# strongbeamsprout/gloria-nlp-project

Hardware: AMD Instinct MI355X
Metric: image-text pairs/sec (whole node), imagenome_pretrain bs=256 (higher is better)
Workload: dtype bf16

## Files before the change

gloria-nlp-project_amd/csrc/glr_attn.hip:

```cpp
#include "glr_attn_common.h"

namespace {

__global__ void __launch_bounds__(AT_NT) k_attn_fwd(AttnParams p) {
  extern __shared__ __attribute__((aligned(16))) unsigned char smem[];
  const int tid = threadIdx.x, lane = tid & 63, wave = tid >> 6, l31 = lane & 31, h = lane >> 5;
  const int bh = blockIdx.x, b = bh / p.nh, hd = bh % p.nh;
  const int L = p.L, tp = p.tp, lk = (L + 15) & ~15, kt = lk >> 4, nkb = (L + 31) >> 5;
  unsigned char* Qs = smem;
  unsigned char* Ks = Qs + 128 * AT_RP;
  unsigned char* Vt = Ks + 128 * AT_RP;
  unsigned char* Ps = smem;
  float* kb = reinterpret_cast<float*>(Vt + 64 * tp);
  const size_t base = (size_t)b * L * p.ld + (size_t)hd * 64;
  {
    uint4 rq[4], rk[4], rv[4];
    tile_load(p.q + base, p.ld, L, rq, tid);
    tile_load(p.k + base, p.ld, L, rk, tid);
    tile_load(p.v + base, p.ld, L, rv, tid);
    tile_store_rows(rq, Qs, tid);
    tile_store_rows(rk, Ks, tid);
    tile_store_transposed(rv, lk, Vt, tp, tid);
  }
  if (tid < 128) kb[tid] = (tid < L && (p.key_mask == nullptr || p.key_mask[(size_t)b * L + tid] != 0)) ? 0.f : -INFINITY;
  __syncthreads();
  const int row0 = 32 * wave;
  f32x16 acc[4];
#pragma unroll
  for (int j = 0; j < 4; ++j) zero16(acc[j]);
  if (row0 < L) gemm_rows64(acc, Qs, row0, Ks, nkb, l31, h);
  __syncthreads();
  if (row0 >= L) return;
  float kbv[4];
#pragma unroll
  for (int j = 0; j < 4; ++j) kbv[j] = kb[32 * j + l31];
  const bool drop = p.p_drop > 0.f;
  const unsigned thr16 = drop ? (unsigned)(p.p_drop * 65536.f + 0.5f) : 0u;
  const float inv_keep = drop ? 1.f / (1.f - p.p_drop) : 1.f;
  const float sl = p.scale * AT_LOG2E;
  unsigned char* slab = Ps + wave * 32 * AT_SP;
  unsigned mw0 = 0u, mw1 = 0u;
  unsigned hk0, hk1;
  hash_key(p, hk0, hk1);
#pragma unroll
  for (int q = 0; q < 16; ++q) {
    const int r = acc_row(q, h);
    float v[4], m = -INFINITY;
#pragma unroll
    for (int j = 0; j < 4; ++j) { v[j] = __builtin_fmaf(acc[j][q], sl, kbv[j]); m = fmaxf(m, v[j]); }
    m = half_max(m);
    const float ms = m == -INFINITY ? 0.f : m;
    float e[4], s = 0.f;
#pragma unroll
    for (int j = 0; j < 4; ++j) { e[j] = __builtin_amdgcn_exp2f(v[j] - ms); s += e[j]; }
    s = half_sum(s);
    const float inv = s > 0.f ? 1.f / s : 0.f;
    if (l31 == 0) p.lse[(size_t)bh * 128 + row0 + r] = (ms + __builtin_amdgcn_logf(fmaxf(s, 1e-37f))) * (1.f / AT_LOG2E);
    unsigned r01 = 0u, r23 = 0u;
    if (drop) {
      const unsigned ctr = (((unsigned)bh * 128u + (unsigned)(row0 + r)) * 32u + (unsigned)l31) * 2u;
      r01 = hash32(ctr, hk0, hk1);
      r23 = hash32(ctr + 1u, hk0, hk1);
    }
    const unsigned r16[4] = {r01 & 0xffffu, r01 >> 16, r23 & 0xffffu, r23 >> 16};
#pragma unroll
    for (int j = 0; j < 4; ++j) {
      const bool keepb = !drop || r16[j] >= thr16;
      if (drop) {
        const unsigned long long word = __ballot(keepb);
        if (lane == q * 4 + j) { mw0 = (unsigned)word; mw1 = (unsigned)(word >> 32); }
      }
      const float pd = keepb ? e[j] * inv * inv_keep : 0.f;
      *reinterpret_cast<unsigned short*>(slab + r * AT_SP + (32 * j + l31) * 2) = f2bf(pd);
    }
  }
  if (drop) {
    const int q = lane >> 2, j = lane & 3;
    const int r0 = row0 + acc_row(q, 0);
    p.keep[((size_t)bh * 128 + r0) * 4 + j] = mw0;
    p.keep[((size_t)bh * 128 + r0 + 4) * 4 + j] = mw1;
  }
  f32x16 out[2];
  zero16(out[0]); zero16(out[1]);
  gemm_tokens(out, slab, Vt, tp, kt, l31, h);
  store_rows(out, slab, tp, p.o + (size_t)b * L * p.ld_o + (size_t)hd * 64, p.ld_o, row0, L, lane, l31, h);
}

__global__ void __launch_bounds__(AT_NT, 2) k_attn_bwd_q(AttnParams p) {
  extern __shared__ __attribute__((aligned(16))) unsigned char smem[];
  const int tid = threadIdx.x, lane = tid & 63, wave = tid >> 6, l31 = lane & 31, h = lane >> 5;
  const int bh = blockIdx.x, b = bh / p.nh, hd = bh % p.nh;
  const int L = p.L, tp = p.tp, lk = (L + 15) & ~15, kt = lk >> 4, nkb = (L + 31) >> 5;
  unsigned char* Ks = smem;
  unsigned char* Vs = Ks + 128 * AT_RP;
  unsigned char* Kt = Vs + 128 * AT_RP;
  unsigned char* Ps = smem;
  float* kb = reinterpret_cast<float*>(Kt + 64 * tp);
  float* lse = kb + 128;
  float* delta = lse + 128;
  unsigned* keep = reinterpret_cast<unsigned*>(delta + 128);
  const size_t base = (size_t)b * L * p.ld + (size_t)hd * 64, base_o = (size_t)b * L * p.ld_o + (size_t)hd * 64;
  const bool drop = p.p_drop > 0.f;
  const int row0 = 32 * wave;
  const bool active = row0 < L;
  bf16x8 fq[4], fg[4];
  {
    uint4 rk[4], rv[4];
    bf16x8 fo[4];
    tile_load(p.k + base, p.ld, L, rk, tid);
    tile_load(p.v + base, p.ld, L, rv, tid);
    frag_rows_load(p.q + base, p.ld, row0 + l31, L, h, fq);
    frag_rows_load(p.d_o + base_o, p.ld_o, row0 + l31, L, h, fg);
    frag_rows_load(p.o + base_o, p.ld_o, row0 + l31, L, h, fo);
    if (tid < 128) {
      kb[tid] = (tid < L && (p.key_mask == nullptr || p.key_mask[(size_t)b * L + tid] != 0)) ? 0.f : -INFINITY;
      lse[tid] = tid < L ? p.lse[(size_t)bh * 128 + tid] * AT_LOG2E : 0.f;
    }
    for (int i = tid; i < 512; i += AT_NT) keep[i] = (drop && (i >> 2) < L) ? p.keep[(size_t)bh * 512 + i] : 0xffffffffu;
    tile_store_rows(rk, Ks, tid);
    tile_store_rows(rv, Vs, tid);
    tile_store_transposed(rk, lk, Kt, tp, tid);
    float d = 0.f;
#pragma unroll
    for (int ks = 0; ks < 4; ++ks) d += dot8(__builtin_bit_cast(uint4, fg[ks]), __builtin_bit_cast(uint4, fo[ks]));
    d += __shfl_xor(d, 32, 64);
    if (h == 0) delta[row0 + l31] = d;
  }
  __syncthreads();
  f32x16 acc[4], acc2[4], out[2];
#pragma unroll
  for (int j = 0; j < 4; ++j) { zero16(acc[j]); zero16(acc2[j]); }
  if (active) {
    gemm_frag64(acc, fq, Ks, nkb, l31, h);
    gemm_frag64(acc2, fg, Vs, nkb, l31, h);
  }
  __syncthreads();
  if (!active) return;
  const float inv_keep = drop ? 1.f / (1.f - p.p_drop) : 1.f;
  const float sl = p.scale * AT_LOG2E;
  unsigned char* slab = Ps + wave * 32 * AT_SP;
  {
    float kbv[4];
#pragma unroll
    for (int j = 0; j < 4; ++j) kbv[j] = kb[32 * j + l31];
#pragma unroll
    for (int q = 0; q < 16; ++q) {
      const int r = acc_row(q, h);
      const float lr = lse[row0 + r], dl = delta[row0 + r];
      const uint4 kw = *reinterpret_cast<const uint4*>(keep + (row0 + r) * 4);
      const unsigned kwj[4] = {kw.x, kw.y, kw.z, kw.w};
#pragma unroll
      for (int j = 0; j < 4; ++j) {
        const float pr = __builtin_amdgcn_exp2f(__builtin_fmaf(acc[j][q], sl, kbv[j]) - lr);
        const float dp = ((kwj[j] >> l31) & 1u) ? acc2[j][q] * inv_keep : 0.f;
        *reinterpret_cast<unsigned short*>(slab + r * AT_SP + (32 * j + l31) * 2) = f2bf(pr * (dp - dl) * p.scale);
      }
    }
  }
  zero16(out[0]); zero16(out[1]);
  gemm_tokens(out, slab, Kt, tp, kt, l31, h);
  store_rows(out, slab, tp, p.dq + base, p.ld, row0, L, lane, l31, h);
}

__global__ void __launch_bounds__(AT_NT, 2) k_attn_bwd_kv(AttnParams p) {
  extern __shared__ __attribute__((aligned(16))) unsigned char smem[];
  const int tid = threadIdx.x, lane = tid & 63, wave = tid >> 6, l31 = lane & 31, h = lane >> 5;
  const int bh = blockIdx.x, b = bh / p.nh, hd = bh % p.nh;
  const int L = p.L, tp = p.tp, lk = (L + 15) & ~15, kt = lk >> 4, nkb = (L + 31) >> 5;
  unsigned char* Qs = smem;
  unsigned char* Gs = Qs + 128 * AT_RP;
  unsigned char* Qt = Gs + 128 * AT_RP;
  unsigned char* Gt = Qt + 64 * tp;
  unsigned char* Ps = smem;
  float* kb = reinterpret_cast<float*>(Gt + 64 * tp);
  float* lse = kb + 128;
  float* delta = lse + 128;
  unsigned* keep = reinterpret_cast<unsigned*>(delta + 256);
  const size_t base = (size_t)b * L * p.ld + (size_t)hd * 64, base_o = (size_t)b * L * p.ld_o + (size_t)hd * 64;
  const bool drop = p.p_drop > 0.f;
  const int row0 = 32 * wave;
  const bool active = row0 < L;
  bf16x8 fk[4], fv[4];
  {
    uint4 rq[4], rg[4], ro[4];
    tile_load(p.q + base, p.ld, L, rq, tid);
    tile_load(p.d_o + base_o, p.ld_o, L, rg, tid);
    tile_load(p.o + base_o, p.ld_o, L, ro, tid);
    frag_rows_load(p.k + base, p.ld, row0 + l31, L, h, fk);
    frag_rows_load(p.v + base, p.ld, row0 + l31, L, h, fv);
    if (tid < 128) {
      kb[tid] = (tid < L && (p.key_mask == nullptr || p.key_mask[(size_t)b * L + tid] != 0)) ? 0.f : -INFINITY;
      lse[tid] = tid < L ? p.lse[(size_t)bh * 128 + tid] * AT_LOG2E : 0.f;
    }
    for (int i = tid; i < 512; i += AT_NT) keep[i] = (drop && (i >> 2) < L) ? p.keep[(size_t)bh * 512 + i] : 0xffffffffu;
    tile_store_rows(rq, Qs, tid);
    tile_store_rows(rg, Gs, tid);
    tile_store_transposed(rq, lk, Qt, tp, tid);
    tile_store_transposed(rg, lk, Gt, tp, tid);
    delta[tid] = (dot8(rg[0], ro[0]) + dot8(rg[1], ro[1])) + (dot8(rg[2], ro[2]) + dot8(rg[3], ro[3]));
  }
  __syncthreads();
  f32x16 acc[4], acc2[4], out[2];
#pragma unroll
  for (int j = 0; j < 4; ++j) { zero16(acc[j]); zero16(acc2[j]); }
  float lq[4], dq_[4], kbk16[16];
  unsigned kwq[4];
  if (active) {
    gemm_frag64(acc, fk, Qs, nkb, l31, h);
    gemm_frag64(acc2, fv, Gs, nkb, l31, h);
  }
#pragma unroll
  for (int j = 0; j < 4; ++j) {
    lq[j] = lse[32 * j + l31];
    dq_[j] = delta[32 * j + l31] + delta[128 + 32 * j + l31];
    kwq[j] = keep[(32 * j + l31) * 4 + wave];
  }
#pragma unroll
  for (int q = 0; q < 16; ++q) kbk16[q] = kb[row0 + acc_row(q, h)];
  __syncthreads();
  if (!active) return;
  const float inv_keep = drop ? 1.f / (1.f - p.p_drop) : 1.f;
  const float sl = p.scale * AT_LOG2E;
  unsigned char* slab = Ps + wave * 32 * AT_SP;
#pragma unroll
  for (int q = 0; q < 16; ++q) {
    const int r = acc_row(q, h);
#pragma unroll
    for (int j = 0; j < 4; ++j) {
      const float pr = __builtin_amdgcn_exp2f(__builtin_fmaf(acc[j][q], sl, kbk16[q]) - lq[j]);
      const bool keepb = (kwq[j] >> r) & 1u;
      *reinterpret_cast<unsigned short*>(slab + r * AT_SP + (32 * j + l31) * 2) = f2bf(keepb ? pr * inv_keep : 0.f);
      const float dp = keepb ? acc2[j][q] * inv_keep : 0.f;
      acc2[j][q] = pr * (dp - dq_[j]) * p.scale;
    }
  }
  zero16(out[0]); zero16(out[1]);
  gemm_tokens(out, slab, Gt, tp, kt, l31, h);
  {
    f32x16 dvv[2] = {out[0], out[1]};
#pragma unroll
    for (int q = 0; q < 16; ++q) {
      const int r = acc_row(q, h);
#pragma unroll
      for (int j = 0; j < 4; ++j) *reinterpret_cast<unsigned short*>(slab + r * AT_SP + (32 * j + l31) * 2) = f2bf(acc2[j][q]);
    }
    zero16(out[0]); zero16(out[1]);
    gemm_tokens(out, slab, Qt, tp, kt, l31, h);
    store_rows(out, slab, tp, p.dk + base, p.ld, row0, L, lane, l31, h);
    store_rows(dvv, slab, tp, p.dv + base, p.ld, row0, L, lane, l31, h);
  }
}

size_t attn_lds_fwd(int L) { return (size_t)2 * 128 * AT_RP + (size_t)64 * attn_tp(L) + 512; }
size_t attn_lds_bwd_q(int L) { return (size_t)2 * 128 * AT_RP + (size_t)64 * attn_tp(L) + 3 * 512 + 2048; }
size_t attn_lds_bwd_kv(int L) { return (size_t)2 * 128 * AT_RP + (size_t)2 * 64 * attn_tp(L) + 4 * 512 + 2048; }
size_t attn_lds_bwd(int L) { return attn_lds_bwd_kv(L) > attn_lds_bwd_q(L) ? attn_lds_bwd_kv(L) : attn_lds_bwd_q(L); }

}

extern "C" int glr_attn_max_tokens(int backward) {
  for (int L = 128; L > 0; L -= 16)
    if ((backward ? attn_lds_bwd(L) : attn_lds_fwd(L)) <= 160 * 1024) return L;
  return 0;
}

extern "C" int glr_attn_fwd(const void* q, const void* k, const void* v, const uint8_t* key_mask, int B, int n_heads, int L, int ld,
                            int ld_o, float scale, float p_drop, unsigned long long seed, unsigned long long offset,
                            const unsigned long long* rng_cell, void* o, float* lse, uint32_t* keep, void* stream) {
  AttnParams p;
  const int rc = attn_fill(p, q, k, v, key_mask, B, n_heads, L, ld, ld_o, scale, p_drop, seed, offset, 128);
  if (rc != GLR_OK) return rc;
  if (!o || !lse || (p_drop > 0.f && !keep) || L > glr_attn_max_tokens(0)) return GLR_EINVAL;
  p.o = (unsigned short*)o; p.lse = lse; p.keep = keep; p.rng = rng_cell;
  const int lds = (int)attn_lds_fwd(L);
  static GlrLdsAttr lds_fwd;
  if (glr_ensure_lds(lds_fwd, (const void*)k_attn_fwd, lds) != GLR_OK) return GLR_ELAUNCH;
  hipLaunchKernelGGL(k_attn_fwd, dim3(B * n_heads), dim3(AT_NT), lds, (hipStream_t)stream, p);
  GLR_CHECK_LAUNCH();
  return GLR_OK;
}

extern "C" int glr_attn_bwd(const void* q, const void* k, const void* v, const void* o, const void* d_o, const uint8_t* key_mask,
                            const float* lse, const uint32_t* keep, int B, int n_heads, int L, int ld, int ld_o, float scale, float p_drop,
                            void* dq, void* dk, void* dv, void* stream) {
  AttnParams p;
  const int rc = attn_fill(p, q, k, v, key_mask, B, n_heads, L, ld, ld_o, scale, p_drop, 0, 0, 128);
  if (rc != GLR_OK) return rc;
  if (!o || !d_o || !lse || !dq || !dk || !dv || (p_drop > 0.f && !keep) || L > glr_attn_max_tokens(1)) return GLR_EINVAL;
  p.o = (unsigned short*)const_cast<void*>(o); p.d_o = (const unsigned short*)d_o; p.lse = const_cast<float*>(lse);
  p.keep = const_cast<unsigned*>(keep); p.dq = (unsigned short*)dq; p.dk = (unsigned short*)dk; p.dv = (unsigned short*)dv;
  const int lds_q = (int)attn_lds_bwd_q(L), lds_kv = (int)attn_lds_bwd_kv(L);
  static GlrLdsAttr lds_bq, lds_bkv;
  if (glr_ensure_lds(lds_bq, (const void*)k_attn_bwd_q, lds_q) != GLR_OK) return GLR_ELAUNCH;
  if (glr_ensure_lds(lds_bkv, (const void*)k_attn_bwd_kv, lds_kv) != GLR_OK) return GLR_ELAUNCH;
  hipLaunchKernelGGL(k_attn_bwd_q, dim3(B * n_heads), dim3(AT_NT), lds_q, (hipStream_t)stream, p);
  GLR_CHECK_LAUNCH();
  hipLaunchKernelGGL(k_attn_bwd_kv, dim3(B * n_heads), dim3(AT_NT), lds_kv, (hipStream_t)stream, p);
  GLR_CHECK_LAUNCH();
  return GLR_OK;
}
```

gloria-nlp-project_amd/csrc/glr_attn_common.h:

```cpp
#pragma once
#include "glr_common.h"

namespace {

constexpr int AT_NT = 256;
constexpr int AT_RP = 144;
constexpr int AT_SP = 272;
constexpr float AT_LOG2E = 1.4426950408889634f;

struct AttnParams {
  const unsigned short* q; const unsigned short* k; const unsigned short* v;
  const unsigned char* key_mask;
  int B, nh, L, ld, ld_o;
  float scale, p_drop;
  unsigned seed_lo, seed_hi, off_lo, off_hi;
  const unsigned long long* rng;
  unsigned short* o;
  float* lse;
  unsigned* keep;
  const unsigned short* d_o;
  unsigned short* dq; unsigned short* dk; unsigned short* dv;
  int tp;
};

__device__ __forceinline__ unsigned mix32(unsigned x) {
  x ^= x >> 16; x *= 0x7feb352du; x ^= x >> 15; x *= 0x846ca68bu; x ^= x >> 16;
  return x;
}
__device__ __forceinline__ unsigned hash32(unsigned ctr, unsigned k0, unsigned k1) { return mix32(mix32(ctr ^ k0) + k1); }

template <int CTRL>
__device__ __forceinline__ float dpp(float v) {
  return __builtin_bit_cast(float, __builtin_amdgcn_update_dpp(0, __builtin_bit_cast(int, v), CTRL, 0xf, 0xf, true));
}
__device__ __forceinline__ float half_max(float v) {
  v = fmaxf(v, dpp<0xB1>(v));
  v = fmaxf(v, dpp<0x4E>(v));
  v = fmaxf(v, dpp<0x141>(v));
  v = fmaxf(v, dpp<0x140>(v));
  return fmaxf(v, __shfl_xor(v, 16, 64));
}
__device__ __forceinline__ float half_sum(float v) {
  v += dpp<0xB1>(v);
  v += dpp<0x4E>(v);
  v += dpp<0x141>(v);
  v += dpp<0x140>(v);
  return v + __shfl_xor(v, 16, 64);
}

__device__ __forceinline__ bf16x8 ldf(const unsigned char* p) { return __builtin_bit_cast(bf16x8, *reinterpret_cast<const uint4*>(p)); }
__device__ __forceinline__ void mma(const bf16x8& a, const bf16x8& b, f32x16& c) { c = __builtin_amdgcn_mfma_f32_32x32x16_bf16(a, b, c, 0, 0, 0); }
__device__ __forceinline__ void zero16(f32x16& a) {
#pragma unroll
  for (int q = 0; q < 16; ++q) a[q] = 0.f;
}
__device__ __forceinline__ int acc_row(int q, int h) { return (q & 3) + 8 * (q >> 2) + 4 * h; }

__device__ __forceinline__ void tile_load(const unsigned short* g, int ld, int L, uint4 (&r)[4], int tid) {
#pragma unroll
  for (int t = 0; t < 4; ++t) {
    const int i = tid + AT_NT * t, row = i & 127, pc = i >> 7;
    r[t] = make_uint4(0u, 0u, 0u, 0u);
    if (row < L) r[t] = *reinterpret_cast<const uint4*>(g + (size_t)row * ld + pc * 8);
  }
}
__device__ __forceinline__ void tile_store_rows(const uint4 (&r)[4], unsigned char* dst, int tid) {
#pragma unroll
  for (int t = 0; t < 4; ++t) {
    const int i = tid + AT_NT * t, row = i & 127, pc = i >> 7;
    *reinterpret_cast<uint4*>(dst + row * AT_RP + pc * 16) = r[t];
  }
}
__device__ __forceinline__ void tile_store_transposed(const uint4 (&r)[4], int lk, unsigned char* dst, int tp, int tid) {
#pragma unroll
  for (int t = 0; t < 4; ++t) {
    const int i = tid + AT_NT * t, row = i & 127, pc = i >> 7;
    if (row < lk) {
      const unsigned w[4] = {r[t].x, r[t].y, r[t].z, r[t].w};
#pragma unroll
      for (int e = 0; e < 4; ++e) {
        *reinterpret_cast<unsigned short*>(dst + (pc * 8 + 2 * e) * tp + row * 2) = (unsigned short)(w[e] & 0xffffu);
        *reinterpret_cast<unsigned short*>(dst + (pc * 8 + 2 * e + 1) * tp + row * 2) = (unsigned short)(w[e] >> 16);
      }
    }
  }
}
__device__ __forceinline__ float dot8(const uint4 a, const uint4 c) {
  const unsigned aw[4] = {a.x, a.y, a.z, a.w}, cw[4] = {c.x, c.y, c.z, c.w};
  float d = 0.f;
#pragma unroll
  for (int e = 0; e < 4; ++e) {
    d = __builtin_fmaf(__uint_as_float(aw[e] << 16), __uint_as_float(cw[e] << 16), d);
    d = __builtin_fmaf(__uint_as_float(aw[e] & 0xffff0000u), __uint_as_float(cw[e] & 0xffff0000u), d);
  }
  return d;
}
__device__ __forceinline__ void gemm_rows64(f32x16 (&acc)[4], const unsigned char* A, int arow0, const unsigned char* Bm, int nblk,
                                            int l31, int h) {
#pragma unroll
  for (int ks = 0; ks < 4; ++ks) {
    const bf16x8 fa = ldf(A + (arow0 + l31) * AT_RP + ks * 32 + h * 16);
#pragma unroll
    for (int j = 0; j < 4; ++j)
      if (j < nblk) mma(fa, ldf(Bm + (32 * j + l31) * AT_RP + ks * 32 + h * 16), acc[j]);
  }
}
__device__ __forceinline__ void gemm_tokens(f32x16 (&out)[2], const unsigned char* slab, const unsigned char* Bt, int tp, int kt,
                                            int l31, int h) {
  for (int ks = 0; ks < kt; ++ks) {
    const bf16x8 fa = ldf(slab + l31 * AT_SP + ks * 32 + h * 16);
#pragma unroll
    for (int c = 0; c < 2; ++c) mma(fa, ldf(Bt + (32 * c + l31) * tp + ks * 32 + h * 16), out[c]);
  }
}
__device__ __forceinline__ void store_rows(const f32x16 (&out)[2], unsigned char* slab, int tp, unsigned short* g, int ld, int row0, int L,
                                           int lane, int l31, int h) {
#pragma unroll
  for (int c = 0; c < 2; ++c)
#pragma unroll
    for (int q = 0; q < 16; ++q)
      *reinterpret_cast<unsigned short*>(slab + acc_row(q, h) * AT_SP + (32 * c + l31) * 2) = f2bf(out[c][q]);
#pragma unroll
  for (int t = 0; t < 4; ++t) {
    const int i = lane + 64 * t, row = i >> 3, pc = i & 7;
    if (row0 + row < L)
      *reinterpret_cast<uint4*>(g + (size_t)(row0 + row) * ld + pc * 8) = *reinterpret_cast<const uint4*>(slab + row * AT_SP + pc * 16);
  }
}

__device__ __forceinline__ void frag_rows_load(const unsigned short* g, int ld, int row, int L, int h, bf16x8 (&f)[4]) {
#pragma unroll
  for (int ks = 0; ks < 4; ++ks) {
    uint4 v = make_uint4(0u, 0u, 0u, 0u);
    if (row < L) v = *reinterpret_cast<const uint4*>(g + (size_t)row * ld + ks * 16 + h * 8);
    f[ks] = __builtin_bit_cast(bf16x8, v);
  }
}
__device__ __forceinline__ void gemm_frag64(f32x16 (&acc)[4], const bf16x8 (&fa)[4], const unsigned char* Bm, int nblk, int l31, int h) {
#pragma unroll
  for (int ks = 0; ks < 4; ++ks)
#pragma unroll
    for (int j = 0; j < 4; ++j)
      if (j < nblk) mma(fa[ks], ldf(Bm + (32 * j + l31) * AT_RP + ks * 32 + h * 16), acc[j]);
}

__device__ __forceinline__ void hash_key(const AttnParams& p, unsigned& hk0, unsigned& hk1) {
  unsigned sd_lo = p.seed_lo, sd_hi = p.seed_hi, of_lo = p.off_lo, of_hi = p.off_hi;
  if (p.rng != nullptr) {
    const unsigned long long s = p.rng[0], o = p.rng[1] + (((unsigned long long)p.off_hi << 32) | p.off_lo);
    sd_lo = (unsigned)s; sd_hi = (unsigned)(s >> 32); of_lo = (unsigned)o; of_hi = (unsigned)(o >> 32);
  }
  hk0 = sd_lo ^ (of_lo * 0x9E3779B9u); hk1 = sd_hi ^ (of_hi * 0x85EBCA6Bu) ^ 0xC2B2AE35u;
}

inline int attn_tp(int L) { return 2 * ((L + 15) & ~15) + 16; }

inline int attn_fill(AttnParams& p, const void* q, const void* k, const void* v, const unsigned char* key_mask, int B, int nh, int L, int ld,
                     int ld_o, float scale, float p_drop, unsigned long long seed, unsigned long long offset, int max_L) {
  if (!q || !k || !v || B <= 0 || nh <= 0 || L <= 0 || L > max_L || ld < nh * 64 || ld % 8 != 0 || ld_o < nh * 64 || ld_o % 8 != 0)
    return GLR_EINVAL;
  if (p_drop < 0.f || p_drop >= 1.f) return GLR_EINVAL;
  p.q = (const unsigned short*)q; p.k = (const unsigned short*)k; p.v = (const unsigned short*)v; p.key_mask = key_mask;
  p.B = B; p.nh = nh; p.L = L; p.ld = ld; p.ld_o = ld_o; p.scale = scale; p.p_drop = p_drop;
  p.seed_lo = (unsigned)seed; p.seed_hi = (unsigned)(seed >> 32); p.off_lo = (unsigned)offset; p.off_hi = (unsigned)(offset >> 32);
  p.rng = nullptr;
  p.o = nullptr; p.lse = nullptr; p.keep = nullptr; p.d_o = nullptr; p.dq = p.dk = p.dv = nullptr;
  p.tp = attn_tp(L < 128 ? L : 128);
  return GLR_OK;
}

}
```

gloria-nlp-project_amd/csrc/glr_attn_long.hip:

```cpp
#include "glr_attn_common.h"

namespace {

constexpr int AL_MAX = 512;
constexpr int AL_TP = 272;

__device__ __forceinline__ float key_bias(const AttnParams& p, int b, int key) {
  return (key < p.L && (p.key_mask == nullptr || p.key_mask[(size_t)b * p.L + key] != 0)) ? 0.f : -INFINITY;
}
__device__ __forceinline__ void key_bias_fill(const AttnParams& p, int b, int Lp, float* kb, int* last64, int tid) {
  for (int i0 = 0; i0 < Lp; i0 += AT_NT) {
    const int i = i0 + tid;
    const float v = i < Lp ? key_bias(p, b, i) : -INFINITY;
    const unsigned long long live = __ballot(v == 0.f);
    if (i < Lp) {
      kb[i] = v;
      if ((tid & 63) == 0) last64[i >> 6] = live ? 63 - __builtin_clzll(live) : -1;
    }
  }
}
__device__ __forceinline__ int live_subblocks(const int* last64, int c) {
  const int lo = last64[2 * c], hi = last64[2 * c + 1];
  return hi >= 0 ? (64 + hi) / 32 + 1 : lo >= 0 ? lo / 32 + 1 : 0;
}
__device__ __forceinline__ void uniform_branch() { asm volatile(""); }

__device__ __forceinline__ void keep_load(const AttnParams& p, int bh, int Lp, int qb, int kc, unsigned (&w)[2], int tid) {
#pragma unroll
  for (int t = 0; t < 2; ++t) {
    const int i = tid + AT_NT * t, row = qb * 128 + (i >> 2);
    w[t] = (p.p_drop > 0.f && row < p.L) ? p.keep[((size_t)bh * Lp + row) * (Lp >> 5) + kc * 4 + (i & 3)] : 0xffffffffu;
  }
}

__global__ void __launch_bounds__(AT_NT, 2) k_attn_long_fwd(AttnParams p) {
  extern __shared__ __attribute__((aligned(16))) unsigned char smem[];
  const int tid = threadIdx.x, lane = tid & 63, wave = tid >> 6, l31 = lane & 31, h = lane >> 5;
  const int L = p.L, Lp = (L + 127) & ~127, nb = Lp >> 7;
  const int bh = blockIdx.x / nb, qb = blockIdx.x % nb, b = bh / p.nh, hd = bh % p.nh;
  unsigned char* Ks = smem;
  unsigned char* Vt = Ks + 128 * AT_RP;
  unsigned char* Ps = Vt + 64 * AL_TP;
  float* kb = reinterpret_cast<float*>(Ps + 128 * AT_SP);
  int* last64 = reinterpret_cast<int*>(kb + AL_MAX);
  const size_t base = (size_t)b * L * p.ld + (size_t)hd * 64;
  const int row0 = qb * 128 + 32 * wave;
  const bool active = row0 < L;
  bf16x8 fq[4];
  frag_rows_load(p.q + base, p.ld, row0 + l31, L, h, fq);
  key_bias_fill(p, b, Lp, kb, last64, tid);
  __syncthreads();
  const float sl = p.scale * AT_LOG2E;
  float m[16], s[16];
#pragma unroll
  for (int q = 0; q < 16; ++q) { m[q] = -INFINITY; s[q] = 0.f; }
  for (int c = 0; c < nb; ++c) {
    const int ne = live_subblocks(last64, c);
    if (ne == 0) continue;
    uint4 rk[4];
    tile_load(p.k + base + (size_t)c * 128 * p.ld, p.ld, min(L - c * 128, 32 * ne), rk, tid);
    __syncthreads();
    tile_store_rows(rk, Ks, tid);
    __syncthreads();
    if (active) {
      f32x16 acc[4];
#pragma unroll
      for (int j = 0; j < 4; ++j) zero16(acc[j]);
      gemm_frag64(acc, fq, Ks, ne, l31, h);
      float kbv[4];
#pragma unroll
      for (int j = 0; j < 4; ++j) kbv[j] = kb[c * 128 + 32 * j + l31];
#pragma unroll
      for (int q = 0; q < 16; ++q) {
        float v[4], mb = -INFINITY;
#pragma unroll
        for (int j = 0; j < 4; ++j)
          if (j < ne) { uniform_branch(); v[j] = __builtin_fmaf(acc[j][q], sl, kbv[j]); mb = fmaxf(mb, v[j]); }
        const float mn = fmaxf(m[q], half_max(mb));
        const float ms = mn == -INFINITY ? 0.f : mn;
        float e = 0.f;
#pragma unroll
        for (int j = 0; j < 4; ++j)
          if (j < ne) { uniform_branch(); e += __builtin_amdgcn_exp2f(v[j] - ms); }
        s[q] = __builtin_fmaf(s[q], __builtin_amdgcn_exp2f(m[q] - ms), half_sum(e));
        m[q] = mn;
      }
    }
  }
  const bool drop = p.p_drop > 0.f;
  const unsigned thr16 = drop ? (unsigned)(p.p_drop * 65536.f + 0.5f) : 0u;
  const float inv_keep = drop ? 1.f / (1.f - p.p_drop) : 1.f;
  if (active) {
#pragma unroll
    for (int q = 0; q < 16; ++q) {
      const float ms = m[q] == -INFINITY ? 0.f : m[q];
      if (l31 == 0)
        p.lse[(size_t)bh * Lp + row0 + acc_row(q, h)] = (ms + __builtin_amdgcn_logf(fmaxf(s[q], 1e-37f))) * (1.f / AT_LOG2E);
      m[q] = ms;
      s[q] = s[q] > 0.f ? 1.f / s[q] : 0.f;
    }
  }
  unsigned hk0, hk1;
  hash_key(p, hk0, hk1);
  unsigned char* slab = Ps + wave * 32 * AT_SP;
  f32x16 out[2];
  zero16(out[0]); zero16(out[1]);
  for (int c = 0; c < nb; ++c) {
    const int ne = live_subblocks(last64, c);
    if (ne == 0) continue;
    const int rem = min(L - c * 128, 32 * ne), lk = (rem + 15) & ~15;
    uint4 rk[4], rv[4];
    tile_load(p.k + base + (size_t)c * 128 * p.ld, p.ld, rem, rk, tid);
    tile_load(p.v + base + (size_t)c * 128 * p.ld, p.ld, rem, rv, tid);
    __syncthreads();
    tile_store_rows(rk, Ks, tid);
    tile_store_transposed(rv, lk, Vt, AL_TP, tid);
    __syncthreads();
    if (active) {
      f32x16 acc[4];
#pragma unroll
      for (int j = 0; j < 4; ++j) zero16(acc[j]);
      gemm_frag64(acc, fq, Ks, ne, l31, h);
      float kbv[4];
#pragma unroll
      for (int j = 0; j < 4; ++j) kbv[j] = kb[c * 128 + 32 * j + l31];
      unsigned mw0 = 0u, mw1 = 0u;
#pragma unroll
      for (int q = 0; q < 16; ++q) {
        const int r = acc_row(q, h);
        unsigned r01 = 0u, r23 = 0u;
        if (drop) {
          const unsigned ctr = ((((unsigned)bh * (unsigned)AL_MAX + (unsigned)(row0 + r)) * 4u + (unsigned)c) * 32u + (unsigned)l31) * 2u;
          r01 = hash32(ctr, hk0, hk1);
          r23 = hash32(ctr + 1u, hk0, hk1);
        }
        const unsigned r16[4] = {r01 & 0xffffu, r01 >> 16, r23 & 0xffffu, r23 >> 16};
#pragma unroll
        for (int j = 0; j < 4; ++j) {
          if (j >= ne) continue;
          const float e = __builtin_amdgcn_exp2f(__builtin_fmaf(acc[j][q], sl, kbv[j]) - m[q]);
          const bool keepb = !drop || r16[j] >= thr16;
          if (drop) {
            const unsigned long long word = __ballot(keepb);
            if (lane == q * 4 + j) { mw0 = (unsigned)word; mw1 = (unsigned)(word >> 32); }
          }
          const float pd = keepb ? e * s[q] * inv_keep : 0.f;
          *reinterpret_cast<unsigned short*>(slab + r * AT_SP + (32 * j + l31) * 2) = f2bf(pd);
        }
      }
      if (drop && (lane & 3) < ne) {
        const int q = lane >> 2, j = lane & 3;
        const size_t w0 = ((size_t)bh * Lp + row0 + acc_row(q, 0)) * (Lp >> 5) + c * 4 + j;
        p.keep[w0] = mw0;
        p.keep[w0 + 4 * (Lp >> 5)] = mw1;
      }
      gemm_tokens(out, slab, Vt, AL_TP, lk >> 4, l31, h);
    }
  }
  if (active) store_rows(out, slab, AL_TP, p.o + (size_t)b * L * p.ld_o + (size_t)hd * 64, p.ld_o, row0, L, lane, l31, h);
}

__global__ void __launch_bounds__(AT_NT, 2) k_attn_long_bwd_q(AttnParams p) {
  extern __shared__ __attribute__((aligned(16))) unsigned char smem[];
  const int tid = threadIdx.x, lane = tid & 63, wave = tid >> 6, l31 = lane & 31, h = lane >> 5;
  const int L = p.L, Lp = (L + 127) & ~127, nb = Lp >> 7;
  const int bh = blockIdx.x / nb, qb = blockIdx.x % nb, b = bh / p.nh, hd = bh % p.nh;
  unsigned char* Ks = smem;
  unsigned char* Vs = Ks + 128 * AT_RP;
  unsigned char* Kt = Vs + 128 * AT_RP;
  unsigned char* Ps = smem;
  float* kb = reinterpret_cast<float*>(Kt + 64 * AL_TP);
  float* lse = kb + AL_MAX;
  float* delta = lse + 128;
  unsigned* keep = reinterpret_cast<unsigned*>(delta + 128);
  int* last64 = reinterpret_cast<int*>(keep + 512);
  const size_t base = (size_t)b * L * p.ld + (size_t)hd * 64, base_o = (size_t)b * L * p.ld_o + (size_t)hd * 64;
  const int row0 = qb * 128 + 32 * wave;
  const bool active = row0 < L;
  bf16x8 fq[4];
  {
    bf16x8 fg[4], fo[4];
    frag_rows_load(p.q + base, p.ld, row0 + l31, L, h, fq);
    frag_rows_load(p.d_o + base_o, p.ld_o, row0 + l31, L, h, fg);
    frag_rows_load(p.o + base_o, p.ld_o, row0 + l31, L, h, fo);
    key_bias_fill(p, b, Lp, kb, last64, tid);
    if (tid < 128) lse[tid] = qb * 128 + tid < L ? p.lse[(size_t)bh * Lp + qb * 128 + tid] * AT_LOG2E : 0.f;
    float d = 0.f;
#pragma unroll
    for (int ks = 0; ks < 4; ++ks) d += dot8(__builtin_bit_cast(uint4, fg[ks]), __builtin_bit_cast(uint4, fo[ks]));
    d += __shfl_xor(d, 32, 64);
    if (h == 0) delta[32 * wave + l31] = d;
  }
  __syncthreads();
  const bool drop = p.p_drop > 0.f;
  const float inv_keep = drop ? 1.f / (1.f - p.p_drop) : 1.f;
  const float sl = p.scale * AT_LOG2E;
  unsigned char* slab = Ps + wave * 32 * AT_SP;
  f32x16 out[2];
  zero16(out[0]); zero16(out[1]);
  for (int c = 0; c < nb; ++c) {
    const int ne = live_subblocks(last64, c);
    if (ne == 0) continue;
    const int rem = min(L - c * 128, 32 * ne), lk = (rem + 15) & ~15;
    bf16x8 fg[4];
    frag_rows_load(p.d_o + base_o, p.ld_o, row0 + l31, L, h, fg);
    {
      uint4 rk[4], rv[4];
      unsigned kw[2];
      tile_load(p.k + base + (size_t)c * 128 * p.ld, p.ld, rem, rk, tid);
      tile_load(p.v + base + (size_t)c * 128 * p.ld, p.ld, rem, rv, tid);
      keep_load(p, bh, Lp, qb, c, kw, tid);
      __syncthreads();
      tile_store_rows(rk, Ks, tid);
      tile_store_rows(rv, Vs, tid);
      tile_store_transposed(rk, lk, Kt, AL_TP, tid);
      keep[tid] = kw[0]; keep[tid + AT_NT] = kw[1];
    }
    __syncthreads();
    f32x16 acc[4], acc2[4];
#pragma unroll
    for (int j = 0; j < 4; ++j) { zero16(acc[j]); zero16(acc2[j]); }
    if (active) {
      gemm_frag64(acc, fq, Ks, ne, l31, h);
      gemm_frag64(acc2, fg, Vs, ne, l31, h);
    }
    __syncthreads();
    if (active) {
      float kbv[4];
#pragma unroll
      for (int j = 0; j < 4; ++j) kbv[j] = kb[c * 128 + 32 * j + l31];
#pragma unroll
      for (int q = 0; q < 16; ++q) {
        const int r = acc_row(q, h);
        const float lr = lse[32 * wave + r], dl = delta[32 * wave + r];
        const uint4 kw = *reinterpret_cast<const uint4*>(keep + (32 * wave + r) * 4);
        const unsigned kwj[4] = {kw.x, kw.y, kw.z, kw.w};
#pragma unroll
        for (int j = 0; j < 4; ++j) {
          if (j >= ne) continue;
          const float pr = __builtin_amdgcn_exp2f(__builtin_fmaf(acc[j][q], sl, kbv[j]) - lr);
          const float dp = ((kwj[j] >> l31) & 1u) ? acc2[j][q] * inv_keep : 0.f;
          *reinterpret_cast<unsigned short*>(slab + r * AT_SP + (32 * j + l31) * 2) = f2bf(pr * (dp - dl) * p.scale);
        }
      }
      gemm_tokens(out, slab, Kt, AL_TP, lk >> 4, l31, h);
    }
  }
  if (active) store_rows(out, slab, AL_TP, p.dq + base, p.ld, row0, L, lane, l31, h);
}

__global__ void __launch_bounds__(AT_NT, 2) k_attn_long_bwd_kv(AttnParams p) {
  extern __shared__ __attribute__((aligned(16))) unsigned char smem[];
  const int tid = threadIdx.x, lane = tid & 63, wave = tid >> 6, l31 = lane & 31, h = lane >> 5;
  const int L = p.L, Lp = (L + 127) & ~127, nb = Lp >> 7;
  const int bh = blockIdx.x / nb, kc = blockIdx.x % nb, b = bh / p.nh, hd = bh % p.nh;
  unsigned char* Qs = smem;
  unsigned char* Gs = Qs + 128 * AT_RP;
  unsigned char* Qt = Gs + 128 * AT_RP;
  unsigned char* Gt = Qt + 64 * AL_TP;
  unsigned char* Ps = smem;
  float* lse = reinterpret_cast<float*>(Gt + 64 * AL_TP);
  float* delta = lse + 128;
  unsigned* keep = reinterpret_cast<unsigned*>(delta + 256);
  float* kb = reinterpret_cast<float*>(keep + 512);
  const size_t base = (size_t)b * L * p.ld + (size_t)hd * 64, base_o = (size_t)b * L * p.ld_o + (size_t)hd * 64;
  const int row0 = kc * 128 + 32 * wave;
  const bool active = row0 < L;
  const float kbt = tid < 128 ? key_bias(p, b, kc * 128 + tid) : -INFINITY;
  if (tid < 128) kb[tid] = kbt;
  const bool blk_live = __syncthreads_or(kbt == 0.f);
  const bool compute = active && __ballot(kb[32 * wave + l31] == 0.f) != 0ull;
  const bool drop = p.p_drop > 0.f;
  const float inv_keep = drop ? 1.f / (1.f - p.p_drop) : 1.f;
  const float sl = p.scale * AT_LOG2E;
  unsigned char* slab = Ps + wave * 32 * AT_SP;
  f32x16 dk[2], dv[2];
  zero16(dk[0]); zero16(dk[1]); zero16(dv[0]); zero16(dv[1]);
  for (int c = 0; c < (blk_live ? nb : 0); ++c) {
    const int rem = L - c * 128, lk = min(128, (rem + 15) & ~15), nqb = min(4, (rem + 31) >> 5);
    bf16x8 fk[4], fv[4];
    frag_rows_load(p.k + base, p.ld, row0 + l31, L, h, fk);
    frag_rows_load(p.v + base, p.ld, row0 + l31, L, h, fv);
    {
      uint4 rq[4], rg[4], ro[4];
      unsigned kw[2];
      const size_t blk = (size_t)c * 128;
      tile_load(p.q + base + blk * p.ld, p.ld, rem, rq, tid);
      tile_load(p.d_o + base_o + blk * p.ld_o, p.ld_o, rem, rg, tid);
      tile_load(p.o + base_o + blk * p.ld_o, p.ld_o, rem, ro, tid);
      keep_load(p, bh, Lp, c, kc, kw, tid);
      const float lr = (tid < 128 && tid < rem) ? p.lse[(size_t)bh * Lp + c * 128 + tid] * AT_LOG2E : 0.f;
      __syncthreads();
      tile_store_rows(rq, Qs, tid);
      tile_store_rows(rg, Gs, tid);
      tile_store_transposed(rq, lk, Qt, AL_TP, tid);
      tile_store_transposed(rg, lk, Gt, AL_TP, tid);
      keep[tid] = kw[0]; keep[tid + AT_NT] = kw[1];
      if (tid < 128) lse[tid] = lr;
      delta[tid] = (dot8(rg[0], ro[0]) + dot8(rg[1], ro[1])) + (dot8(rg[2], ro[2]) + dot8(rg[3], ro[3]));
    }
    __syncthreads();
    f32x16 acc[4], acc2[4];
#pragma unroll
    for (int j = 0; j < 4; ++j) { zero16(acc[j]); zero16(acc2[j]); }
    float lq[4], dq_[4];
    unsigned kwq[4];
    if (compute) {
      gemm_frag64(acc, fk, Qs, nqb, l31, h);
      gemm_frag64(acc2, fv, Gs, nqb, l31, h);
    }
#pragma unroll
    for (int j = 0; j < 4; ++j) {
      lq[j] = lse[32 * j + l31];
      dq_[j] = delta[32 * j + l31] + delta[128 + 32 * j + l31];
      kwq[j] = keep[(32 * j + l31) * 4 + wave];
    }
    __syncthreads();
    if (compute) {
#pragma unroll
      for (int q = 0; q < 16; ++q) {
        const int r = acc_row(q, h);
        const float kbk = kb[32 * wave + r];
#pragma unroll
        for (int j = 0; j < 4; ++j) {
          if (j >= nqb) continue;
          const float pr = __builtin_amdgcn_exp2f(__builtin_fmaf(acc[j][q], sl, kbk) - lq[j]);
          const bool keepb = (kwq[j] >> r) & 1u;
          *reinterpret_cast<unsigned short*>(slab + r * AT_SP + (32 * j + l31) * 2) = f2bf(keepb ? pr * inv_keep : 0.f);
          const float dp = keepb ? acc2[j][q] * inv_keep : 0.f;
          acc2[j][q] = pr * (dp - dq_[j]) * p.scale;
        }
      }
      gemm_tokens(dv, slab, Gt, AL_TP, lk >> 4, l31, h);
#pragma unroll
      for (int q = 0; q < 16; ++q) {
        const int r = acc_row(q, h);
#pragma unroll
        for (int j = 0; j < 4; ++j)
          if (j < nqb) *reinterpret_cast<unsigned short*>(slab + r * AT_SP + (32 * j + l31) * 2) = f2bf(acc2[j][q]);
      }
      gemm_tokens(dk, slab, Qt, AL_TP, lk >> 4, l31, h);
    }
  }
  if (active) {
    store_rows(dk, slab, AL_TP, p.dk + base, p.ld, row0, L, lane, l31, h);
    store_rows(dv, slab, AL_TP, p.dv + base, p.ld, row0, L, lane, l31, h);
  }
}

constexpr int AL_LDS_FWD = 128 * AT_RP + 64 * AL_TP + 128 * AT_SP + AL_MAX * 4 + 64;
constexpr int AL_LDS_BWD_Q = 2 * 128 * AT_RP + 64 * AL_TP + AL_MAX * 4 + 2 * 512 + 2048 + 64;
constexpr int AL_LDS_BWD_KV = 2 * 128 * AT_RP + 2 * 64 * AL_TP + 4 * 512 + 2048;
static_assert(128 * AT_SP <= 2 * 128 * AT_RP, "the slabs take the place of two row-major operands");
static_assert(AL_LDS_FWD <= 80 * 1024 && AL_LDS_BWD_Q <= 80 * 1024 && AL_LDS_BWD_KV <= 80 * 1024, "two workgroups per CU");

}

extern "C" int glr_attn_long_max_tokens(void) { return AL_MAX; }

extern "C" int glr_attn_long_fwd(const void* q, const void* k, const void* v, const uint8_t* key_mask, int B, int n_heads, int L,
                                 int ld, int ld_o, float scale, float p_drop, unsigned long long seed, unsigned long long offset,
                                 const unsigned long long* rng_cell, void* o, float* lse, uint32_t* keep, void* stream) {
  AttnParams p;
  const int rc = attn_fill(p, q, k, v, key_mask, B, n_heads, L, ld, ld_o, scale, p_drop, seed, offset, AL_MAX);
  if (rc != GLR_OK) return rc;
  if (!o || !lse || (p_drop > 0.f && !keep)) return GLR_EINVAL;
  p.o = (unsigned short*)o; p.lse = lse; p.keep = keep; p.rng = rng_cell;
  static GlrLdsAttr lds_fwd;
  if (glr_ensure_lds(lds_fwd, (const void*)k_attn_long_fwd, AL_LDS_FWD) != GLR_OK) return GLR_ELAUNCH;
  const int nb = (L + 127) >> 7;
  hipLaunchKernelGGL(k_attn_long_fwd, dim3(B * n_heads * nb), dim3(AT_NT), AL_LDS_FWD, (hipStream_t)stream, p);
  GLR_CHECK_LAUNCH();
  return GLR_OK;
}

extern "C" int glr_attn_long_bwd(const void* q, const void* k, const void* v, const void* o, const void* d_o, const uint8_t* key_mask,
                                 const float* lse, const uint32_t* keep, int B, int n_heads, int L, int ld, int ld_o, float scale,
                                 float p_drop, void* dq, void* dk, void* dv, void* stream) {
  AttnParams p;
  const int rc = attn_fill(p, q, k, v, key_mask, B, n_heads, L, ld, ld_o, scale, p_drop, 0, 0, AL_MAX);
  if (rc != GLR_OK) return rc;
  if (!o || !d_o || !lse || !dq || !dk || !dv || (p_drop > 0.f && !keep)) return GLR_EINVAL;
  p.o = (unsigned short*)const_cast<void*>(o); p.d_o = (const unsigned short*)d_o; p.lse = const_cast<float*>(lse);
  p.keep = const_cast<unsigned*>(keep); p.dq = (unsigned short*)dq; p.dk = (unsigned short*)dk; p.dv = (unsigned short*)dv;
  static GlrLdsAttr lds_bq, lds_bkv;
  if (glr_ensure_lds(lds_bq, (const void*)k_attn_long_bwd_q, AL_LDS_BWD_Q) != GLR_OK) return GLR_ELAUNCH;
  if (glr_ensure_lds(lds_bkv, (const void*)k_attn_long_bwd_kv, AL_LDS_BWD_KV) != GLR_OK) return GLR_ELAUNCH;
  const int nb = (L + 127) >> 7;
  hipLaunchKernelGGL(k_attn_long_bwd_q, dim3(B * n_heads * nb), dim3(AT_NT), AL_LDS_BWD_Q, (hipStream_t)stream, p);
  GLR_CHECK_LAUNCH();
  hipLaunchKernelGGL(k_attn_long_bwd_kv, dim3(B * n_heads * nb), dim3(AT_NT), AL_LDS_BWD_KV, (hipStream_t)stream, p);
  GLR_CHECK_LAUNCH();
  return GLR_OK;
}
```

Before: 3330.

## Skip fully masked trailing key blocks in short-sequence attention kernels

Each short-sequence attention kernel (forward, dQ and dK/dV backward) now computes how many 32-key blocks contain live keys, using a ballot over the key mask. K/V loads, the QK and dO·V GEMMs, the softmax/dropout loops and the P·V GEMM are limited to those blocks, and the forward softmax is templated on the block count. In the dK/dV kernel, waves that own only masked keys write zeros and return early. This removes work on padded keys for padded text batches, at the cost of more template instantiations, a branch on block count, and more care needed to keep dropout masks consistent.

```diff
diff --git a/gloria-nlp-project_amd/csrc/glr_attn.hip b/gloria-nlp-project_amd/csrc/glr_attn.hip
--- a/gloria-nlp-project_amd/csrc/glr_attn.hip
+++ b/gloria-nlp-project_amd/csrc/glr_attn.hip
@@ -2,35 +2,9 @@
 
 namespace {
 
-__global__ void __launch_bounds__(AT_NT) k_attn_fwd(AttnParams p) {
-  extern __shared__ __attribute__((aligned(16))) unsigned char smem[];
-  const int tid = threadIdx.x, lane = tid & 63, wave = tid >> 6, l31 = lane & 31, h = lane >> 5;
-  const int bh = blockIdx.x, b = bh / p.nh, hd = bh % p.nh;
-  const int L = p.L, tp = p.tp, lk = (L + 15) & ~15, kt = lk >> 4, nkb = (L + 31) >> 5;
-  unsigned char* Qs = smem;
-  unsigned char* Ks = Qs + 128 * AT_RP;
-  unsigned char* Vt = Ks + 128 * AT_RP;
-  unsigned char* Ps = smem;
-  float* kb = reinterpret_cast<float*>(Vt + 64 * tp);
-  const size_t base = (size_t)b * L * p.ld + (size_t)hd * 64;
-  {
-    uint4 rq[4], rk[4], rv[4];
-    tile_load(p.q + base, p.ld, L, rq, tid);
-    tile_load(p.k + base, p.ld, L, rk, tid);
-    tile_load(p.v + base, p.ld, L, rv, tid);
-    tile_store_rows(rq, Qs, tid);
-    tile_store_rows(rk, Ks, tid);
-    tile_store_transposed(rv, lk, Vt, tp, tid);
-  }
-  if (tid < 128) kb[tid] = (tid < L && (p.key_mask == nullptr || p.key_mask[(size_t)b * L + tid] != 0)) ? 0.f : -INFINITY;
-  __syncthreads();
-  const int row0 = 32 * wave;
-  f32x16 acc[4];
-#pragma unroll
-  for (int j = 0; j < 4; ++j) zero16(acc[j]);
-  if (row0 < L) gemm_rows64(acc, Qs, row0, Ks, nkb, l31, h);
-  __syncthreads();
-  if (row0 >= L) return;
+template <int NE>
+__device__ __forceinline__ void fwd_rows(const AttnParams& p, const f32x16 (&acc)[4], const float* kb, unsigned char* slab, int bh,
+                                         int row0, int lane, int l31, int h) {
   float kbv[4];
 #pragma unroll
   for (int j = 0; j < 4; ++j) kbv[j] = kb[32 * j + l31];
@@ -38,7 +12,6 @@
   const unsigned thr16 = drop ? (unsigned)(p.p_drop * 65536.f + 0.5f) : 0u;
   const float inv_keep = drop ? 1.f / (1.f - p.p_drop) : 1.f;
   const float sl = p.scale * AT_LOG2E;
-  unsigned char* slab = Ps + wave * 32 * AT_SP;
   unsigned mw0 = 0u, mw1 = 0u;
   unsigned hk0, hk1;
   hash_key(p, hk0, hk1);
@@ -47,24 +20,27 @@
     const int r = acc_row(q, h);
     float v[4], m = -INFINITY;
 #pragma unroll
-    for (int j = 0; j < 4; ++j) { v[j] = __builtin_fmaf(acc[j][q], sl, kbv[j]); m = fmaxf(m, v[j]); }
+    for (int j = 0; j < 4; ++j)
+      if (j < NE) { v[j] = __builtin_fmaf(acc[j][q], sl, kbv[j]); m = fmaxf(m, v[j]); }
     m = half_max(m);
     const float ms = m == -INFINITY ? 0.f : m;
     float e[4], s = 0.f;
 #pragma unroll
-    for (int j = 0; j < 4; ++j) { e[j] = __builtin_amdgcn_exp2f(v[j] - ms); s += e[j]; }
+    for (int j = 0; j < 4; ++j)
+      if (j < NE) { e[j] = __builtin_amdgcn_exp2f(v[j] - ms); s += e[j]; }
     s = half_sum(s);
     const float inv = s > 0.f ? 1.f / s : 0.f;
     if (l31 == 0) p.lse[(size_t)bh * 128 + row0 + r] = (ms + __builtin_amdgcn_logf(fmaxf(s, 1e-37f))) * (1.f / AT_LOG2E);
     unsigned r01 = 0u, r23 = 0u;
-    if (drop) {
+    if (drop && NE > 0) {
       const unsigned ctr = (((unsigned)bh * 128u + (unsigned)(row0 + r)) * 32u + (unsigned)l31) * 2u;
       r01 = hash32(ctr, hk0, hk1);
-      r23 = hash32(ctr + 1u, hk0, hk1);
+      if (NE > 2) r23 = hash32(ctr + 1u, hk0, hk1);
     }
     const unsigned r16[4] = {r01 & 0xffffu, r01 >> 16, r23 & 0xffffu, r23 >> 16};
 #pragma unroll
     for (int j = 0; j < 4; ++j) {
+      if (j >= NE) continue;
       const bool keepb = !drop || r16[j] >= thr16;
       if (drop) {
         const unsigned long long word = __ballot(keepb);
@@ -74,12 +50,54 @@
       *reinterpret_cast<unsigned short*>(slab + r * AT_SP + (32 * j + l31) * 2) = f2bf(pd);
     }
   }
-  if (drop) {
+  if (drop && (lane & 3) < NE) {
     const int q = lane >> 2, j = lane & 3;
     const int r0 = row0 + acc_row(q, 0);
     p.keep[((size_t)bh * 128 + r0) * 4 + j] = mw0;
     p.keep[((size_t)bh * 128 + r0 + 4) * 4 + j] = mw1;
   }
+}
+
+__global__ void __launch_bounds__(AT_NT) k_attn_fwd(AttnParams p) {
+  extern __shared__ __attribute__((aligned(16))) unsigned char smem[];
+  const int tid = threadIdx.x, lane = tid & 63, wave = tid >> 6, l31 = lane & 31, h = lane >> 5;
+  const int bh = blockIdx.x, b = bh / p.nh, hd = bh % p.nh;
+  const int L = p.L, tp = p.tp;
+  unsigned char* Qs = smem;
+  unsigned char* Ks = Qs + 128 * AT_RP;
+  unsigned char* Vt = Ks + 128 * AT_RP;
+  unsigned char* Ps = smem;
+  float* kb = reinterpret_cast<float*>(Vt + 64 * tp);
+  const size_t base = (size_t)b * L * p.ld + (size_t)hd * 64;
+  float kb0, kb1;
+  const int ne = key_blocks(p, b, lane, kb0, kb1);
+  const int Lk = min(L, 32 * ne), lk = (Lk + 15) & ~15, kt = lk >> 4;
+  {
+    uint4 rq[4], rk[4], rv[4];
+    tile_load(p.q + base, p.ld, L, rq, tid);
+    tile_load(p.k + base, p.ld, Lk, rk, tid);
+    tile_load(p.v + base, p.ld, Lk, rv, tid);
+    tile_store_rows(rq, Qs, tid);
+    tile_store_rows(rk, Ks, tid);
+    tile_store_transposed(rv, lk, Vt, tp, tid);
+  }
+  if (wave == 0) { kb[lane] = kb0; kb[64 + lane] = kb1; }
+  __syncthreads();
+  const int row0 = 32 * wave;
+  f32x16 acc[4];
+#pragma unroll
+  for (int j = 0; j < 4; ++j) zero16(acc[j]);
+  if (row0 < L) gemm_rows64(acc, Qs, row0, Ks, ne, l31, h);
+  __syncthreads();
+  if (row0 >= L) return;
+  unsigned char* slab = Ps + wave * 32 * AT_SP;
+  switch (ne) {
+    case 0: fwd_rows<0>(p, acc, kb, slab, bh, row0, lane, l31, h); break;
+    case 1: fwd_rows<1>(p, acc, kb, slab, bh, row0, lane, l31, h); break;
+    case 2: fwd_rows<2>(p, acc, kb, slab, bh, row0, lane, l31, h); break;
+    case 3: fwd_rows<3>(p, acc, kb, slab, bh, row0, lane, l31, h); break;
+    default: fwd_rows<4>(p, acc, kb, slab, bh, row0, lane, l31, h); break;
+  }
   f32x16 out[2];
   zero16(out[0]); zero16(out[1]);
   gemm_tokens(out, slab, Vt, tp, kt, l31, h);
@@ -90,7 +108,7 @@
   extern __shared__ __attribute__((aligned(16))) unsigned char smem[];
   const int tid = threadIdx.x, lane = tid & 63, wave = tid >> 6, l31 = lane & 31, h = lane >> 5;
   const int bh = blockIdx.x, b = bh / p.nh, hd = bh % p.nh;
-  const int L = p.L, tp = p.tp, lk = (L + 15) & ~15, kt = lk >> 4, nkb = (L + 31) >> 5;
+  const int L = p.L, tp = p.tp;
   unsigned char* Ks = smem;
   unsigned char* Vs = Ks + 128 * AT_RP;
   unsigned char* Kt = Vs + 128 * AT_RP;
@@ -103,20 +121,22 @@
   const bool drop = p.p_drop > 0.f;
   const int row0 = 32 * wave;
   const bool active = row0 < L;
+  float kb0, kb1;
+  const int ne = key_blocks(p, b, lane, kb0, kb1);
+  const int Lk = min(L, 32 * ne), lk = (Lk + 15) & ~15, kt = lk >> 4;
   bf16x8 fq[4], fg[4];
   {
     uint4 rk[4], rv[4];
     bf16x8 fo[4];
-    tile_load(p.k + base, p.ld, L, rk, tid);
-    tile_load(p.v + base, p.ld, L, rv, tid);
+    tile_load(p.k + base, p.ld, Lk, rk, tid);
+    tile_load(p.v + base, p.ld, Lk, rv, tid);
     frag_rows_load(p.q + base, p.ld, row0 + l31, L, h, fq);
     frag_rows_load(p.d_o + base_o, p.ld_o, row0 + l31, L, h, fg);
     frag_rows_load(p.o + base_o, p.ld_o, row0 + l31, L, h, fo);
-    if (tid < 128) {
-      kb[tid] = (tid < L && (p.key_mask == nullptr || p.key_mask[(size_t)b * L + tid] != 0)) ? 0.f : -INFINITY;
-      lse[tid] = tid < L ? p.lse[(size_t)bh * 128 + tid] * AT_LOG2E : 0.f;
-    }
-    for (int i = tid; i < 512; i += AT_NT) keep[i] = (drop && (i >> 2) < L) ? p.keep[(size_t)bh * 512 + i] : 0xffffffffu;
+    if (wave == 0) { kb[lane] = kb0; kb[64 + lane] = kb1; }
+    if (tid < 128) lse[tid] = tid < L ? p.lse[(size_t)bh * 128 + tid] * AT_LOG2E : 0.f;
+    for (int i = tid; i < 512; i += AT_NT)
+      keep[i] = (drop && (i >> 2) < L && (i & 3) < ne) ? p.keep[(size_t)bh * 512 + i] : 0xffffffffu;
     tile_store_rows(rk, Ks, tid);
     tile_store_rows(rv, Vs, tid);
     tile_store_transposed(rk, lk, Kt, tp, tid);
@@ -131,8 +151,8 @@
 #pragma unroll
   for (int j = 0; j < 4; ++j) { zero16(acc[j]); zero16(acc2[j]); }
   if (active) {
-    gemm_frag64(acc, fq, Ks, nkb, l31, h);
-    gemm_frag64(acc2, fg, Vs, nkb, l31, h);
+    gemm_frag64(acc, fq, Ks, ne, l31, h);
+    gemm_frag64(acc2, fg, Vs, ne, l31, h);
   }
   __syncthreads();
   if (!active) return;
@@ -151,6 +171,8 @@
       const unsigned kwj[4] = {kw.x, kw.y, kw.z, kw.w};
 #pragma unroll
       for (int j = 0; j < 4; ++j) {
+        if (j >= ne) continue;
+        uniform_branch();
         const float pr = __builtin_amdgcn_exp2f(__builtin_fmaf(acc[j][q], sl, kbv[j]) - lr);
         const float dp = ((kwj[j] >> l31) & 1u) ? acc2[j][q] * inv_keep : 0.f;
         *reinterpret_cast<unsigned short*>(slab + r * AT_SP + (32 * j + l31) * 2) = f2bf(pr * (dp - dl) * p.scale);
@@ -179,20 +201,21 @@
   const size_t base = (size_t)b * L * p.ld + (size_t)hd * 64, base_o = (size_t)b * L * p.ld_o + (size_t)hd * 64;
   const bool drop = p.p_drop > 0.f;
   const int row0 = 32 * wave;
-  const bool active = row0 < L;
+  float kb0, kb1;
+  const int ne = key_blocks(p, b, lane, kb0, kb1);
+  const bool compute = wave < ne;
   bf16x8 fk[4], fv[4];
   {
     uint4 rq[4], rg[4], ro[4];
     tile_load(p.q + base, p.ld, L, rq, tid);
     tile_load(p.d_o + base_o, p.ld_o, L, rg, tid);
     tile_load(p.o + base_o, p.ld_o, L, ro, tid);
-    frag_rows_load(p.k + base, p.ld, row0 + l31, L, h, fk);
-    frag_rows_load(p.v + base, p.ld, row0 + l31, L, h, fv);
-    if (tid < 128) {
-      kb[tid] = (tid < L && (p.key_mask == nullptr || p.key_mask[(size_t)b * L + tid] != 0)) ? 0.f : -INFINITY;
-      lse[tid] = tid < L ? p.lse[(size_t)bh * 128 + tid] * AT_LOG2E : 0.f;
-    }
-    for (int i = tid; i < 512; i += AT_NT) keep[i] = (drop && (i >> 2) < L) ? p.keep[(size_t)bh * 512 + i] : 0xffffffffu;
+    frag_rows_load(p.k + base, p.ld, row0 + l31, compute ? L : 0, h, fk);
+    frag_rows_load(p.v + base, p.ld, row0 + l31, compute ? L : 0, h, fv);
+    if (wave == 0) { kb[lane] = kb0; kb[64 + lane] = kb1; }
+    if (tid < 128) lse[tid] = tid < L ? p.lse[(size_t)bh * 128 + tid] * AT_LOG2E : 0.f;
+    for (int i = tid; i < 512; i += AT_NT)
+      keep[i] = (drop && (i >> 2) < L && (i & 3) < ne) ? p.keep[(size_t)bh * 512 + i] : 0xffffffffu;
     tile_store_rows(rq, Qs, tid);
     tile_store_rows(rg, Gs, tid);
     tile_store_transposed(rq, lk, Qt, tp, tid);
@@ -205,20 +228,24 @@
   for (int j = 0; j < 4; ++j) { zero16(acc[j]); zero16(acc2[j]); }
   float lq[4], dq_[4], kbk16[16];
   unsigned kwq[4];
-  if (active) {
+  if (compute) {
     gemm_frag64(acc, fk, Qs, nkb, l31, h);
     gemm_frag64(acc2, fv, Gs, nkb, l31, h);
-  }
-#pragma unroll
-  for (int j = 0; j < 4; ++j) {
-    lq[j] = lse[32 * j + l31];
-    dq_[j] = delta[32 * j + l31] + delta[128 + 32 * j + l31];
-    kwq[j] = keep[(32 * j + l31) * 4 + wave];
-  }
-#pragma unroll
-  for (int q = 0; q < 16; ++q) kbk16[q] = kb[row0 + acc_row(q, h)];
-  __syncthreads();
-  if (!active) return;
+#pragma unroll
+    for (int j = 0; j < 4; ++j) {
+      lq[j] = lse[32 * j + l31];
+      dq_[j] = delta[32 * j + l31] + delta[128 + 32 * j + l31];
+      kwq[j] = keep[(32 * j + l31) * 4 + wave];
+    }
+#pragma unroll
+    for (int q = 0; q < 16; ++q) kbk16[q] = kb[row0 + acc_row(q, h)];
+  }
+  __syncthreads();
+  if (!compute) {
+    zero_rows(p.dk + base, p.ld, row0, L, lane);
+    zero_rows(p.dv + base, p.ld, row0, L, lane);
+    return;
+  }
   const float inv_keep = drop ? 1.f / (1.f - p.p_drop) : 1.f;
   const float sl = p.scale * AT_LOG2E;
   unsigned char* slab = Ps + wave * 32 * AT_SP;
diff --git a/gloria-nlp-project_amd/csrc/glr_attn_common.h b/gloria-nlp-project_amd/csrc/glr_attn_common.h
--- a/gloria-nlp-project_amd/csrc/glr_attn_common.h
+++ b/gloria-nlp-project_amd/csrc/glr_attn_common.h
@@ -144,6 +144,26 @@
       if (j < nblk) mma(fa[ks], ldf(Bm + (32 * j + l31) * AT_RP + ks * 32 + h * 16), acc[j]);
 }
 
+__device__ __forceinline__ float key_bias(const AttnParams& p, int b, int key) {
+  return (key < p.L && (p.key_mask == nullptr || p.key_mask[(size_t)b * p.L + key] != 0)) ? 0.f : -INFINITY;
+}
+__device__ __forceinline__ int last_live(unsigned long long live) { return live ? 63 - __builtin_clzll(live) : -1; }
+__device__ __forceinline__ int live_blocks(int lo, int hi) { return hi >= 0 ? (64 + hi) / 32 + 1 : lo >= 0 ? lo / 32 + 1 : 0; }
+__device__ __forceinline__ void uniform_branch() { asm volatile(""); }
+__device__ __forceinline__ int key_blocks(const AttnParams& p, int b, int lane, float& kb0, float& kb1) {
+  kb0 = key_bias(p, b, lane);
+  kb1 = key_bias(p, b, 64 + lane);
+  const int lo = last_live(__ballot(kb0 == 0.f)), hi = last_live(__ballot(kb1 == 0.f));
+  return live_blocks(lo, hi);
+}
+__device__ __forceinline__ void zero_rows(unsigned short* g, int ld, int row0, int L, int lane) {
+#pragma unroll
+  for (int t = 0; t < 4; ++t) {
+    const int i = lane + 64 * t, row = i >> 3, pc = i & 7;
+    if (row0 + row < L) *reinterpret_cast<uint4*>(g + (size_t)(row0 + row) * ld + pc * 8) = make_uint4(0u, 0u, 0u, 0u);
+  }
+}
+
 __device__ __forceinline__ void hash_key(const AttnParams& p, unsigned& hk0, unsigned& hk1) {
   unsigned sd_lo = p.seed_lo, sd_hi = p.seed_hi, of_lo = p.off_lo, of_hi = p.off_hi;
   if (p.rng != nullptr) {
diff --git a/gloria-nlp-project_amd/csrc/glr_attn_long.hip b/gloria-nlp-project_amd/csrc/glr_attn_long.hip
--- a/gloria-nlp-project_amd/csrc/glr_attn_long.hip
+++ b/gloria-nlp-project_amd/csrc/glr_attn_long.hip
@@ -5,9 +5,6 @@
 constexpr int AL_MAX = 512;
 constexpr int AL_TP = 272;
 
-__device__ __forceinline__ float key_bias(const AttnParams& p, int b, int key) {
-  return (key < p.L && (p.key_mask == nullptr || p.key_mask[(size_t)b * p.L + key] != 0)) ? 0.f : -INFINITY;
-}
 __device__ __forceinline__ void key_bias_fill(const AttnParams& p, int b, int Lp, float* kb, int* last64, int tid) {
   for (int i0 = 0; i0 < Lp; i0 += AT_NT) {
     const int i = i0 + tid;
@@ -15,15 +12,11 @@
     const unsigned long long live = __ballot(v == 0.f);
     if (i < Lp) {
       kb[i] = v;
-      if ((tid & 63) == 0) last64[i >> 6] = live ? 63 - __builtin_clzll(live) : -1;
-    }
-  }
-}
-__device__ __forceinline__ int live_subblocks(const int* last64, int c) {
-  const int lo = last64[2 * c], hi = last64[2 * c + 1];
-  return hi >= 0 ? (64 + hi) / 32 + 1 : lo >= 0 ? lo / 32 + 1 : 0;
-}
-__device__ __forceinline__ void uniform_branch() { asm volatile(""); }
+      if ((tid & 63) == 0) last64[i >> 6] = last_live(live);
+    }
+  }
+}
+__device__ __forceinline__ int live_subblocks(const int* last64, int c) { return live_blocks(last64[2 * c], last64[2 * c + 1]); }
 
 __device__ __forceinline__ void keep_load(const AttnParams& p, int bh, int Lp, int qb, int kc, unsigned (&w)[2], int tid) {
 #pragma unroll
```

Result: no change. 3353, median of 6 (+0.7%).
